# ManuelZ/image-search-engine

Measured on AMD Instinct MI355X. Metric: queries/sec, exact brute-force L2 kNN (recall@10 vs exact CPU), 1Mx512 fp32 index, k=10, higher is better.
Workload: dtype f32; 1 GPU; 1000000x512 fp32 uniform[0,1) index (default_rng 1234), L2, k=10, nq=16 queries per step, index resident in HBM, steps issued round-robin on 16 HIP streams; 400 untimed steps ahead of the warm-up bring the GPU out of its idle power state; n=1000000, d=512, k=10, nq=16

## Files before the change

image-search-engine_amd/_native.py:

```python
from __future__ import annotations

import ctypes
import os

import torch

_HERE = os.path.dirname(os.path.abspath(__file__))
LIB_PATH = os.environ.get("ISE_KNN_LIB") or os.path.join(_HERE, "csrc", "libise_knn.so")

METRIC_INNER_PRODUCT = 0
METRIC_L2 = 1
MAX_K = 2048
PQ_MAX_M = 64
SQ_MAX_D = 2048
SQ_8BIT, SQ_8BIT_UNIFORM = 0, 2
STORE_F32, STORE_BF16 = 0, 1

E_INVALID, E_HIP, E_NOMEM, E_NODEVICE = -1, -2, -3, -4

_f32p = ctypes.POINTER(ctypes.c_float)
_i64p = ctypes.POINTER(ctypes.c_int64)
_u64p = ctypes.POINTER(ctypes.c_uint64)
_vp = ctypes.c_void_p
_i64 = ctypes.c_int64
_int = ctypes.c_int
PROTOTYPES = [
    ("ise_version", _int, []),
    ("ise_last_error", ctypes.c_char_p, []),
    ("ise_device_count", _int, [ctypes.POINTER(_int)]),
    ("ise_device_arch", _int, [_int, ctypes.c_char_p, _int]),
    ("ise_index_create", _int, [ctypes.POINTER(_vp), _int, _int, _int]),
    ("ise_index_create_ex", _int, [ctypes.POINTER(_vp), _int, _int, _int, _int]),
    ("ise_index_destroy", _int, [_vp]),
    ("ise_index_reset", _int, [_vp]),
    ("ise_index_info", _int, [_vp, ctypes.POINTER(_int), ctypes.POINTER(_int), _i64p, ctypes.POINTER(_int)]),
    ("ise_index_set_shift", _int, [_vp, _vp]),
    ("ise_index_get_shift", _int, [_vp, _vp]),
    ("ise_index_stats", _int, [_vp, _u64p]),
    ("ise_index_host_stats", _int, [_vp, _u64p]),
    ("ise_index_reserve_workspaces", _int, [_vp, _i64, _int]),
    ("ise_index_add_host", _int, [_vp, _vp, _i64]),
    ("ise_index_add_device", _int, [_vp, _vp, _i64, _vp]),
    ("ise_index_reconstruct_host", _int, [_vp, _i64, _i64, _vp]),
    ("ise_index_search_host", _int, [_vp, _vp, _i64, _int, _vp, _vp]),
    ("ise_index_search_device", _int, [_vp, _vp, _i64, _int, _vp, _vp, _vp]),
    ("ise_index_search_keys_device", _int, [_vp, _vp, _i64, _int, ctypes.c_uint32, _vp, _vp]),
    ("ise_index_assign_device", _int, [_vp, _vp, _i64, _vp, _vp, _vp]),
    ("ise_merge_keys_device", _int, [_vp, _int, _i64, _int, _int, _vp, _vp, _int, _vp]),
    ("ise_normalize_rows_device", _int, [_vp, _i64, _int, _int, _vp]),
    ("ise_normalize_rows_host", _int, [_vp, _i64, _int, _int]),
    ("ise_bovw_histogram_device", _int, [_vp, _vp, _i64, _int, _vp, _int, _vp]),
    ("ise_index_short_stats", _int, [_vp, _vp]),
    ("ise_index_half_stats", _int, [_vp, _u64p]),
    ("ise_index_shadow_row", _int, [_vp, _i64, _f32p]),
    ("ise_index_byte_stats", _int, [_vp, _u64p]),
    ("ise_index_depth_stats", _int, [_vp, _u64p]),
    ("ise_index_byte_row", _int, [_vp, _i64, _f32p]),
    ("ise_index_stage_query_debug", _int, [_vp, _vp, _int, _vp, _i64, _f32p, ctypes.POINTER(ctypes.c_int32)]),
    ("ise_index_range_search_host", _int, [_vp, _vp, _i64, ctypes.c_float, ctypes.POINTER(_vp)]),
    ("ise_range_result_get", _int, [_vp, _i64p, ctypes.POINTER(_vp), ctypes.POINTER(_vp), ctypes.POINTER(_vp)]),
    ("ise_range_result_destroy", _int, [_vp]),
    ("ise_index_range_stats", _int, [_vp, _u64p]),
    ("ise_index_remove_ids_host", _int, [_vp, _vp, _i64, _i64p]),
    ("ise_index_remove_range", _int, [_vp, _i64, _i64, _i64p]),
    ("ise_index_remove_stats", _int, [_vp, _u64p]),
    ("ise_index_remove_last_timing", _int, [_vp, _f32p, _u64p]),
    ("ise_selector_create_range", _int, [_vp, _i64, _i64, ctypes.POINTER(_vp)]),
    ("ise_selector_create_ids", _int, [_vp, _vp, _i64, _int, ctypes.POINTER(_vp)]),
    ("ise_selector_create_bitmap", _int, [_vp, _vp, _i64, ctypes.POINTER(_vp)]),
    ("ise_selector_info", _int, [_vp, _i64p]),
    ("ise_selector_destroy", _int, [_vp]),
    ("ise_index_search_sel_device", _int, [_vp, _vp, _i64, _int, _vp, _vp, _vp, _vp]),
    ("ise_index_search_sel_host", _int, [_vp, _vp, _i64, _int, _vp, _vp, _vp]),
    ("ise_index_range_search_sel_host", _int, [_vp, _vp, _i64, ctypes.c_float, _vp, ctypes.POINTER(_vp)]),
    ("ise_index_sel_stats", _int, [_vp, _u64p]),
    ("ise_index_search_subset_device", _int, [_vp, _vp, _i64, _int, _vp, _int, _vp, _vp, _vp]),
    ("ise_index_search_subset_host", _int, [_vp, _vp, _i64, _int, _vp, _int, _vp, _vp]),
    ("ise_index_distance_subset_device", _int, [_vp, _vp, _i64, _vp, _int, _vp, _vp]),
    ("ise_index_distance_subset_host", _int, [_vp, _vp, _i64, _vp, _int, _vp]),
    ("ise_index_subset_stats", _int, [_vp, _u64p]),
    ("ise_binary_index_create", _int, [ctypes.POINTER(_vp), _int, _int]),
    ("ise_binary_index_destroy", _int, [_vp]),
    ("ise_binary_index_reset", _int, [_vp]),
    ("ise_binary_index_info", _int, [_vp, ctypes.POINTER(_int), _i64p, ctypes.POINTER(_int)]),
    ("ise_binary_index_add_host", _int, [_vp, _vp, _i64]),
    ("ise_binary_index_add_device", _int, [_vp, _vp, _i64, _vp]),
    ("ise_binary_index_reconstruct_host", _int, [_vp, _i64, _i64, _vp]),
    ("ise_binary_index_search_host", _int, [_vp, _vp, _i64, _int, _vp, _vp]),
    ("ise_binary_index_search_device", _int, [_vp, _vp, _i64, _int, _vp, _vp, _vp]),
    ("ise_binary_index_range_search_host", _int, [_vp, _vp, _i64, ctypes.c_int32, ctypes.POINTER(_vp)]),
    ("ise_binary_range_result_get", _int, [_vp, _i64p, ctypes.POINTER(_vp), ctypes.POINTER(_vp), ctypes.POINTER(_vp)]),
    ("ise_binary_range_result_destroy", _int, [_vp]),
    ("ise_binary_index_stats", _int, [_vp, _u64p]),
    ("ise_binary_index_remove_ids_host", _int, [_vp, _vp, _i64, _i64p]),
    ("ise_binary_index_remove_range", _int, [_vp, _i64, _i64, _i64p]),
    ("ise_binary_index_remove_stats", _int, [_vp, _u64p]),
    ("ise_binary_selector_create_range", _int, [_vp, _i64, _i64, ctypes.POINTER(_vp)]),
    ("ise_binary_selector_create_ids", _int, [_vp, _vp, _i64, _int, ctypes.POINTER(_vp)]),
    ("ise_binary_selector_create_bitmap", _int, [_vp, _vp, _i64, ctypes.POINTER(_vp)]),
    ("ise_binary_selector_info", _int, [_vp, _i64p]),
    ("ise_binary_selector_destroy", _int, [_vp]),
    ("ise_binary_index_search_sel_host", _int, [_vp, _vp, _i64, _int, _vp, _vp, _vp]),
    ("ise_binary_index_search_sel_device", _int, [_vp, _vp, _i64, _int, _vp, _vp, _vp, _vp]),
    ("ise_binary_index_range_search_sel_host", _int, [_vp, _vp, _i64, ctypes.c_int32, _vp, ctypes.POINTER(_vp)]),
    ("ise_binary_index_sel_stats", _int, [_vp, _u64p]),
    ("ise_ivf_create", _int, [ctypes.POINTER(_vp), _int, _int, _int, _int]),
    ("ise_ivf_destroy", _int, [_vp]),
    ("ise_ivf_reset", _int, [_vp]),
    ("ise_ivf_info", _int, [_vp, ctypes.POINTER(_int), ctypes.POINTER(_int), ctypes.POINTER(_int), _i64p, ctypes.POINTER(_int)]),
    ("ise_ivf_add_host", _int, [_vp, _vp, _vp, _i64]),
# ... 82 lines not shown
```

image-search-engine_amd/csrc/ise_knn.hip:

```cpp

#include "ise_host.hpp"
#include "ise_geometry.hpp"
#include "ise_scan_params.hpp"
#include "ise_assign.hpp"
#include "ise_exact.hpp"
#include "ise_merge.hpp"
#include "ise_exact_scan.hpp"
#include "ise_gemm_scan.hpp"
#include "ise_gemm_bf16.hpp"
#include "ise_rows.hpp"
#include "ise_short_scan.hpp"
#include "ise_range.hpp"
#include "ise_sel_scan.hpp"
#include "ise_stage.hpp"
#include "ise_remove.hpp"
#include "ise_remove_plan.hpp"
#include "ise_selector.hpp"
#include "ise_subset.hpp"

static thread_local std::string g_err;
int ise_fail_(int code, const std::string& msg) {
    g_err = msg;
    return code;
}
// ... 280 lines not shown
    }
    h->xb = h->norms = nullptr;
    h->n = h->cap = 0;
}

extern "C" int ise_index_destroy(ise_index_t* h) {
    if (!h) return ISE_OK;
    {
        DeviceGuard gd(h->device);
        (void)hipDeviceSynchronize();
        free_all(h);
        if (h->mu) (void)hipFree(h->mu);
        if (h->stats_dev) (void)hipFree(h->stats_dev);
        if (h->stream) (void)hipStreamDestroy(h->stream);
    }
    delete h;
    return ISE_OK;
}

extern "C" int ise_index_reset(ise_index_t* h) {
    if (!h) return fail(ISE_E_INVALID, "handle is NULL");
    std::lock_guard<std::mutex> lk(h->mu_);
    DeviceGuard gd(h->device);
    HIP_TRY(hipDeviceSynchronize());
    if (h->xb) (void)hipFree(h->xb);
    if (h->norms) (void)hipFree(h->norms);
    free_shadow(h);
    h->shadow_off = false;
    h->byte_off = false;
    if (h->n > 0) h->row_epoch++;
    h->xb = h->norms = nullptr;
    h->n = h->cap = 0;
    h->shift_pinned = false;
    h->mu_rows = h->norms_rows = 0;
    HIP_TRY(hipMemset(h->mu, 0, (size_t)h->dp * sizeof(float)));
    return ISE_OK;
}

extern "C" int ise_index_info(const ise_index_t* h, int* d, int* metric, int64_t* ntotal, int* device) {
    if (!h) return fail(ISE_E_INVALID, "handle is NULL");
    if (d) *d = h->d;
    if (metric) *metric = h->metric;
    if (ntotal) *ntotal = h->n;
    if (device) *device = h->device;
    return ISE_OK;
}

static int reserve_rows(ise_index* h, long long need, hipStream_t st) {
    if (need <= h->cap) return ISE_OK;
    long long cap = h->cap ? h->cap : 0;
    long long want = need;
    if (cap > 0 && want < cap + cap / 2) want = cap + cap / 2;
    want = (want + 15) / 16 * 16;
    const size_t rb = row_bytes(h);
    char* nx = nullptr;
    float* nn = nullptr;
    HIP_TRY(hipMalloc(&nx, (size_t)want * rb));
    hipError_t e = hipMalloc(&nn, (size_t)want * sizeof(float));
    if (e != hipSuccess) {
        (void)hipFree(nx);
        return fail(ISE_E_NOMEM, std::string("hipMalloc(norms): ") + hipGetErrorString(e));
    }
    if (h->n > 0) {
        HIP_TRY(hipMemcpyAsync(nx, h->xb, (size_t)h->n * rb, hipMemcpyDeviceToDevice, st));
        HIP_TRY(hipMemcpyAsync(nn, h->norms, (size_t)h->n * sizeof(float), hipMemcpyDeviceToDevice, st));
    }
    HIP_TRY(hipMemsetAsync(nx + (size_t)h->n * rb, 0, (size_t)(want - h->n) * rb, st));
    HIP_TRY(hipMemsetAsync(nn + h->n, 0, (size_t)(want - h->n) * sizeof(float), st));
    char* nxh = nullptr;
    float* nmeta = nullptr;
    if (h->xh) {
        const size_t hb = shadow_row_bytes(h);
        if (hipMalloc(&nxh, (size_t)want * hb) != hipSuccess || hipMalloc(&nmeta, (size_t)want * 3 * sizeof(float)) != hipSuccess) {
            (void)hipGetLastError();
            if (nxh) (void)hipFree(nxh);
            nxh = nullptr;
        } else {
            HIP_TRY(hipMemcpyAsync(nxh, h->xh, (size_t)h->n * hb, hipMemcpyDeviceToDevice, st));
            HIP_TRY(hipMemsetAsync(nxh + (size_t)h->n * hb, 0, (size_t)(want - h->n) * hb, st));
            HIP_TRY(hipMemsetAsync(nmeta, 0, (size_t)want * 3 * sizeof(float), st));
            for (int i = 0; i < 3; i++)
                HIP_TRY(hipMemcpyAsync(nmeta + (size_t)i * want, h->hmeta + (size_t)i * h->cap, (size_t)h->n * sizeof(float),
                                       hipMemcpyDeviceToDevice, st));
        }
    }
    char* nxq = nullptr;
    uint32_t* nbm = nullptr;
    if (h->xq8 && nxh) {
        const size_t qb = byte_row_bytes(h);
        if (hipMalloc(&nxq, (size_t)want * qb) != hipSuccess || hipMalloc(&nbm, (size_t)want * sizeof(uint32_t)) != hipSuccess) {
            (void)hipGetLastError();
            if (nxq) (void)hipFree(nxq);
            nxq = nullptr;
        } else {
            HIP_TRY(hipMemcpyAsync(nxq, h->xq8, (size_t)h->n * qb, hipMemcpyDeviceToDevice, st));
            HIP_TRY(hipMemsetAsync(nxq + (size_t)h->n * qb, 0, (size_t)(want - h->n) * qb, st));
            HIP_TRY(hipMemsetAsync(nbm, 0, (size_t)want * sizeof(uint32_t), st));
            HIP_TRY(hipMemcpyAsync(nbm, h->bmeta, (size_t)h->n * sizeof(uint32_t), hipMemcpyDeviceToDevice, st));
        }
    }
    HIP_TRY(hipStreamSynchronize(st));
    if (h->xb) HIP_TRY(hipDeviceSynchronize());
    if (h->xb) (void)hipFree(h->xb);
    if (h->norms) (void)hipFree(h->norms);
    if (h->xh) {
        const bool had_byte = h->xq8 != nullptr;
        free_shadow(h);
        h->shadow_off = nxh == nullptr;
        h->byte_off = h->byte_off || (had_byte && nxh && !nxq);
        h->xh = nxh;
        h->hmeta = nmeta;
        h->xq8 = nxq;
        h->bmeta = nbm;
    }
    h->xb = nx;
    h->norms = nn;
    h->cap = want;
    return ISE_OK;
}

static bool rows_copy_verbatim(const ise_index* h) { return h->storage == ISE_STORE_F32 && h->dp == h->d; }

static bool uses_shift(const ise_index* h) { return h->storage == ISE_STORE_F32 && h->metric == ISE_METRIC_L2; }

static int prepare_shift_locked(ise_index* h, hipStream_t st);

static void launch_shadow(ise_index* h, long long row0, long long n, hipStream_t st) {
    const long long nblk = (n + 3) / 4;
    if (nblk > 0)
        hipLaunchKernelGGL(shadow_rows_kernel, dim3((unsigned)nblk), dim3(256), 0, st, (const float*)h->xb, row0, n, h->d,
                           h->dp, (const float*)h->mu, (_Float16*)h->xh, h->dph, h->hmeta, h->hmeta + h->cap,
                           h->hmeta + 2 * h->cap);
    if (nblk > 0 && h->xq8)
        hipLaunchKernelGGL(byte_rows_kernel, dim3((unsigned)nblk), dim3(256), 0, st, (const float*)h->xb, row0, n, h->d,
                           h->dp, (const float*)h->mu, (int8_t*)h->xq8, h->dpb, h->bmeta);
}

static void launch_norms(ise_index* h, long long row0, long long n, hipStream_t st) {
    const long long nblk = (n + 3) / 4;
    if (h->storage == ISE_STORE_BF16)
        hipLaunchKernelGGL(norms_bf16_kernel, dim3((unsigned)nblk), dim3(256), 0, st, (const __bf16*)h->xb, row0, n,
                           h->dp, h->norms);
    else
        hipLaunchKernelGGL(norms_kernel, dim3((unsigned)nblk), dim3(256), 0, st, (const float*)h->xb, row0, n, h->dp,
                           uses_shift(h) ? h->mu : (const float*)nullptr, h->norms);
    if (h->xh) launch_shadow(h, row0, n, st);
}

#define SHADOW_MIN_ROWS 262144
// ... 1961 lines not shown
    hipEvent_t ev0 = nullptr, ev1 = nullptr;
    ~RemoveScratch() {
        for (void* p : {(void*)g, (void*)cend, (void*)src_idx, (void*)bounce})
            if (p) (void)hipFree(p);
        if (ev0) (void)hipEventDestroy(ev0);
        if (ev1) (void)hipEventDestroy(ev1);
    }
};

static void remove_move_rows(const ise_index* h, void* base, size_t stride, long long a, long long m, const RemoveScratch& sc,
                             hipStream_t st) {
    const uint32_t upr = (uint32_t)(stride / 16);
    const uint32_t total = (uint32_t)(m * upr);
    const uint32_t pieces = (total + 64 * REMOVE_UNROLL - 1) / (64 * REMOVE_UNROLL);
    const unsigned grid = std::max(1u, std::min((pieces + 3) / 4, (unsigned)h->num_cu * 4u));
    hipLaunchKernelGGL(remove_rows_kernel<true>, dim3(grid), dim3(256), 0, st, (const u32x4*)base,
                       (const uint32_t*)sc.src_idx, (u32x4*)sc.bounce, total, upr);
    hipLaunchKernelGGL(remove_rows_kernel<false>, dim3(grid), dim3(256), 0, st, (const u32x4*)sc.bounce,
                       (const uint32_t*)nullptr, (u32x4*)(static_cast<char*>(base) + (size_t)a * stride), total, upr);
}

static int remove_runs_locked(ise_index* h, const std::vector<RemoveRun>& runs, long long removed) {
    const long long n_old = h->n, n_new = n_old - removed, first = runs[0].start;
    const long long moved = n_new - first;
    hipStream_t st = h->stream;
    HIP_TRY(hipDeviceSynchronize());
    if (n_new <= SHADOW_MIN_ROWS) free_shadow(h);
    const bool meta = h->norms_rows == n_old;
    const size_t rb = row_bytes(h), hb = shadow_row_bytes(h), qb = byte_row_bytes(h);
    const bool mv_h = meta && h->xh, mv_q = meta && h->xq8;
    RemoveScratch sc;
    if (moved > 0) {
        const long long T = (long long)runs.size();
        std::vector<uint32_t> g, cend;
        remove_plan_tables(runs, &g, &cend);
        const long long slab = remove_plan_slab_rows(ise_remove_slab_rows_(), (long long)rb, (long long)(rb / 16), moved);
        HIP_TRY(hipMalloc(&sc.g, (size_t)T * sizeof(uint32_t)));
        HIP_TRY(hipMalloc(&sc.cend, (size_t)T * sizeof(uint32_t)));
        HIP_TRY(hipMalloc(&sc.src_idx, (size_t)slab * sizeof(uint32_t)));
        HIP_TRY(hipMalloc(&sc.bounce, (size_t)slab * rb));
        HIP_TRY(hipEventCreate(&sc.ev0));
        HIP_TRY(hipEventCreate(&sc.ev1));
        HIP_TRY(hipMemcpyAsync(sc.g, g.data(), (size_t)T * sizeof(uint32_t), hipMemcpyHostToDevice, st));
        HIP_TRY(hipMemcpyAsync(sc.cend, cend.data(), (size_t)T * sizeof(uint32_t), hipMemcpyHostToDevice, st));
        HIP_TRY(hipStreamSynchronize(st));
        HIP_TRY(hipEventRecord(sc.ev0, st));
        for (long long a = first; a < n_new; a += slab) {
            const long long m = std::min(slab, n_new - a);
            const unsigned gw = (unsigned)std::min<long long>((m + 255) / 256, (long long)h->num_cu * 8);
            hipLaunchKernelGGL(remove_src_kernel, dim3(gw), dim3(256), 0, st, (const uint32_t*)sc.g,
                               (const uint32_t*)sc.cend, (int)T, (uint32_t)a, (uint32_t)m, sc.src_idx);
            remove_move_rows(h, h->xb, rb, a, m, sc, st);
            if (mv_h) remove_move_rows(h, h->xh, hb, a, m, sc, st);
            if (mv_q) remove_move_rows(h, h->xq8, qb, a, m, sc, st);
            if (meta) {
                RemovePlanes gp{}, cp{};
                int np = 0;
                auto plane = [&](void* arr) {
                    uint32_t* w = static_cast<uint32_t*>(arr);
                    uint32_t* b = reinterpret_cast<uint32_t*>(sc.bounce) + (size_t)np * m;
                    gp.src[np] = w;
                    gp.dst[np] = b;
                    cp.src[np] = b;
                    cp.dst[np] = w + a;
                    np++;
                };
                plane(h->norms);
                if (mv_h)
                    for (int i = 0; i < 3; i++) plane(h->hmeta + (size_t)i * h->cap);
                if (mv_q) plane(h->bmeta);
                hipLaunchKernelGGL(remove_words_kernel<true>, dim3(gw, np), dim3(256), 0, st, gp,
                                   (const uint32_t*)sc.src_idx, (uint32_t)m);
                hipLaunchKernelGGL(remove_words_kernel<false>, dim3(gw, np), dim3(256), 0, st, cp,
                                   (const uint32_t*)nullptr, (uint32_t)m);
            }
            HIP_TRY(hipGetLastError());
        }
        HIP_TRY(hipEventRecord(sc.ev1, st));
    }
    HIP_TRY(hipMemsetAsync(static_cast<char*>(h->xb) + (size_t)n_new * rb, 0, (size_t)removed * rb, st));
    HIP_TRY(hipMemsetAsync(h->norms + n_new, 0, (size_t)removed * sizeof(float), st));
    if (h->xh) {
        HIP_TRY(hipMemsetAsync(static_cast<char*>(h->xh) + (size_t)n_new * hb, 0, (size_t)removed * hb, st));
        for (int i = 0; i < 3; i++)
            HIP_TRY(hipMemsetAsync(h->hmeta + (size_t)i * h->cap + n_new, 0, (size_t)removed * sizeof(float), st));
    }
    if (h->xq8) {
        HIP_TRY(hipMemsetAsync(static_cast<char*>(h->xq8) + (size_t)n_new * qb, 0, (size_t)removed * qb, st));
        HIP_TRY(hipMemsetAsync(h->bmeta + n_new, 0, (size_t)removed * sizeof(uint32_t), st));
    }
    h->n = n_new;
    h->row_epoch++;
    h->norms_rows = meta ? n_new : 0;
    const long long mu_rows_old = h->mu_rows;
    h->mu_rows = std::min(h->mu_rows, n_new);
    if (uses_shift(h) && !h->shift_pinned && n_new * 4 < mu_rows_old * 3) h->mu_rows = 0;
    HIP_TRY(hipGetLastError());
    HIP_TRY(hipStreamSynchronize(st));
    h->remove_last_ms = 0.f;
    h->remove_last_bytes = 0;
    if (moved > 0) {
        (void)hipEventElapsedTime(&h->remove_last_ms, sc.ev0, sc.ev1);
        const size_t per_row = rb + (mv_h ? hb + 12 : 0) + (mv_q ? qb + 4 : 0) + (meta ? 4 : 0);
        h->remove_last_bytes = (unsigned long long)moved * per_row;
    }
    h->remove_calls++;
    h->remove_rows += (unsigned long long)removed;
    h->remove_moved += (unsigned long long)moved;
    return ISE_OK;
}

extern "C" int ise_index_remove_range(ise_index_t* h, int64_t i0, int64_t i1, int64_t* n_removed) {
    if (!h) return fail(ISE_E_INVALID, "handle is NULL");
    if (n_removed) *n_removed = 0;
    std::lock_guard<std::mutex> lr(h->rg_mu);
    std::lock_guard<std::mutex> lk(h->mu_);
    const long long a = std::max<long long>(i0, 0), b = std::min<long long>(i1, h->n);
    if (a >= b) return ISE_OK;
    DeviceGuard gd(h->device);
    const int rc = remove_runs_locked(h, {RemoveRun{a, b - a}}, b - a);
    if (rc == ISE_OK && n_removed) *n_removed = b - a;
    return rc;
}

extern "C" int ise_index_remove_ids_host(ise_index_t* h, const int64_t* ids, int64_t n_ids, int64_t* n_removed) {
    if (!h) return fail(ISE_E_INVALID, "handle is NULL");
    if (n_removed) *n_removed = 0;
    if (n_ids < 0 || (n_ids > 0 && !ids)) return fail(ISE_E_INVALID, "ids is NULL");
    if (n_ids == 0) return ISE_OK;
    std::vector<long long> v;
    std::vector<RemoveRun> runs;
    try {
        v = remove_plan_ids(ids, n_ids);
    } catch (const std::bad_alloc&) {
        return fail(ISE_E_NOMEM, "remove_ids: host allocation failed");
    }
    std::lock_guard<std::mutex> lr(h->rg_mu);
    std::lock_guard<std::mutex> lk(h->mu_);
    long long removed = 0;
    try {
        removed = remove_plan_runs(v, h->n, &runs);
// ... 29 lines not shown
    std::lock_guard<std::mutex> lk(h->rg_mu);
    out2[0] = h->range_batches;
    out2[1] = h->range_overflows;
    return ISE_OK;
}

extern "C" int ise_index_short_stats(ise_index_t* h, uint64_t* out1) {
    if (!h || !out1) return fail(ISE_E_INVALID, "NULL argument");
    std::lock_guard<std::mutex> lk(h->mu_);
    out1[0] = h->short_batches;
    return ISE_OK;
}

extern "C" int ise_index_depth_stats(ise_index_t* h, uint64_t* out2) {
    if (!h || !out2) return fail(ISE_E_INVALID, "NULL argument");
    std::lock_guard<std::mutex> lk(h->mu_);
    out2[0] = h->byte_batches - h->byte_deep_batches;
    out2[1] = h->byte_deep_batches;
    return ISE_OK;
}

extern "C" int ise_index_half_stats(ise_index_t* h, uint64_t* out1) {
    if (!h || !out1) return fail(ISE_E_INVALID, "NULL argument");
    std::lock_guard<std::mutex> lk(h->mu_);
    out1[0] = h->half_batches;
    return ISE_OK;
}

extern "C" int ise_index_byte_stats(ise_index_t* h, uint64_t* out2) {
    if (!h || !out2) return fail(ISE_E_INVALID, "NULL argument");
    std::lock_guard<std::mutex> lk(h->mu_);
    out2[0] = h->byte_batches;
    out2[1] = (h->xq8 && byte_rel_ok(h)) ? 1 : 0;
    return ISE_OK;
}

extern "C" int ise_index_byte_row(ise_index_t* h, int64_t i, float* out2) {
    if (!h || !out2) return fail(ISE_E_INVALID, "NULL argument");
    std::lock_guard<std::mutex> lk(h->mu_);
    if (i < 0 || i >= h->n) return fail(ISE_E_INVALID, "row out of range");
    DeviceGuard gd(h->device);
    int rc = prepare_shift_locked(h, h->stream);
    if (rc) return rc;
    if (!h->xq8) return fail(ISE_E_INVALID, "this index has no byte shadow rows");
    HIP_TRY(hipDeviceSynchronize());
    uint32_t m = 0;
    HIP_TRY(hipMemcpy(&m, h->bmeta + i, sizeof(uint32_t), hipMemcpyDeviceToHost));
    uint32_t cb = m << 16, eb = m >> 16;
    float cr;
    memcpy(&cr, &cb, sizeof(float));
    const _Float16 eh = __builtin_bit_cast(_Float16, (unsigned short)eb);
    out2[0] = cr;
    out2[1] = cr * (float)eh;
    return ISE_OK;
}

extern "C" int ise_index_shadow_row(ise_index_t* h, int64_t i, float* out3) {
    if (!h || !out3) return fail(ISE_E_INVALID, "NULL argument");
    std::lock_guard<std::mutex> lk(h->mu_);
    if (i < 0 || i >= h->n) return fail(ISE_E_INVALID, "row out of range");
    DeviceGuard gd(h->device);
    int rc = prepare_shift_locked(h, h->stream);
    if (rc) return rc;
    if (!h->xh) return fail(ISE_E_INVALID, "this index has no shadow rows");
    HIP_TRY(hipDeviceSynchronize());
    for (int j = 0; j < 3; j++)
        HIP_TRY(hipMemcpy(out3 + j, h->hmeta + (size_t)j * h->cap + i, sizeof(float), hipMemcpyDeviceToHost));
    return ISE_OK;
}

extern "C" int ise_index_stage_query_debug(ise_index_t* h, const void* q_dev, int route, void* limbs, int64_t limbs_bytes,
                                           float* out2, int32_t* info3) {
    if (!h || !q_dev || !limbs || !out2 || !info3) return fail(ISE_E_INVALID, "NULL argument");
    if (route != 0 && route != 1) return fail(ISE_E_INVALID, "route: 0 = fp16 shadow, 1 = byte shadow");
    std::lock_guard<std::mutex> lk(h->mu_);
    DeviceGuard gd(h->device);
    int rc = prepare_shift_locked(h, h->stream);
    if (rc) return rc;
    if (route == 1 ? !h->xq8 : !h->xh) return fail(ISE_E_INVALID, "this index has no such shadow rows");
    const int P = route == 1 ? h->dpb : h->dph, es = route == 1 ? 1 : 2;
    const size_t need = (size_t)2 * P * es;
    if (P > 1024 || limbs_bytes < (int64_t)need) return fail(ISE_E_INVALID, "limbs: room for hi and lo of the padded row needed");
    unsigned char* dev = nullptr;
    HIP_TRY(hipMalloc(&dev, need + 16));
    float* out_f = reinterpret_cast<float*>(dev + need);
    int* out_i = reinterpret_cast<int*>(dev + need + 8);
    if (route == 1)
        hipLaunchKernelGGL(stage_debug_kernel<true>, dim3(1), dim3(32), 0, h->stream, (const float*)q_dev, h->mu, h->d, P, dev, out_f, out_i);
    else
        hipLaunchKernelGGL(stage_debug_kernel<false>, dim3(1), dim3(32), 0, h->stream, (const float*)q_dev, h->mu, h->d, P, dev, out_f, out_i);
    hipError_t e = hipGetLastError();
    if (e == hipSuccess) e = hipStreamSynchronize(h->stream);
    std::vector<unsigned char> host(need + 16);
    if (e == hipSuccess) e = hipMemcpy(host.data(), dev, need + 16, hipMemcpyDeviceToHost);
    (void)hipFree(dev);
    HIP_TRY(e);
    memcpy(limbs, host.data(), need);
    memcpy(out2, host.data() + need, 8);
    memcpy(info3, host.data() + need + 8, 8);
    info3[2] = P;
    return ISE_OK;
}

extern "C" int ise_index_host_stats(ise_index_t* h, uint64_t* out3) {
    if (!h || !out3) return fail(ISE_E_INVALID, "NULL argument");
    {
// ... 183 lines not shown
```

image-search-engine_amd/csrc/ise_rows.hpp:

```cpp
#pragma once
#include "ise_common.hpp"

__global__ __launch_bounds__(256) void norms_kernel(const float* __restrict__ x, long long row0,
                                                    long long n, int dp, const float* __restrict__ mu,
                                                    float* __restrict__ out) {
    const int lane = threadIdx.x & 63;
    const long long r = row0 + (long long)blockIdx.x * 4 + (threadIdx.x >> 6);
    if (r >= row0 + n) return;
    const float* xr = x + (size_t)r * dp;
    float s = 0.f;
    for (int j = lane * 4; j < dp; j += 256) {
        const f32x4 x = *reinterpret_cast<const f32x4*>(xr + j);
        f32x4 v = x;
        if (mu) v = v - *reinterpret_cast<const f32x4*>(mu + j);
        s = fmaf(v[0], v[0], s);
        s = fmaf(v[1], v[1], s);
        s = fmaf(v[2], v[2], s);
        s = fmaf(v[3], v[3], s);
        if (mu) s += nonfinite_mark(x);
    }
    s = wave_sum_f32(s);
    if (lane == 0) out[r] = s;
}

__global__ __launch_bounds__(256) void shadow_rows_kernel(const float* __restrict__ x, long long row0, long long n,
                                                          int d, int dp, const float* __restrict__ mu,
                                                          _Float16* __restrict__ xh, int dph, float* __restrict__ hn,
                                                          float* __restrict__ he, float* __restrict__ hs) {
    const int lane = threadIdx.x & 63;
    const long long r = row0 + (long long)blockIdx.x * 4 + (threadIdx.x >> 6);
    if (r >= row0 + n) return;
    const float* xr = x + (size_t)r * dp;
    double amax = 0.0;
    float mark = 0.f;
    for (int j = lane; j < d; j += 64) {
        const float v = xr[j];
        mark += v - v;
        amax = fmax(amax, fabs((double)v - (double)mu[j]));
    }
#pragma unroll
    for (int o = 32; o > 0; o >>= 1) {
        amax = fmax(amax, __shfl_xor(amax, o));
        mark += __shfl_xor(mark, o);
    }
    const bool bad = mark != 0.f;
    const int s = (amax > 0.0 && !bad) ? 14 - ilogb(amax) : 0;
    _Float16* hr = xh + (size_t)r * dph;
    double nu = 0.0, e2 = 0.0;
    for (int j = lane; j < dph; j += 64) {
        const double a = (j < d && !bad) ? (double)xr[j] - (double)mu[j] : 0.0;
        const _Float16 u = (_Float16)(float)ldexp(a, s);
        hr[j] = u;
        const double ut = ldexp((double)(float)u, -s);
        nu = fma(ut, ut, nu);
        e2 = fma(a - ut, a - ut, e2);
    }
#pragma unroll
    for (int o = 32; o > 0; o >>= 1) {
        nu += __shfl_xor(nu, o);
        e2 += __shfl_xor(e2, o);
    }
    if (lane == 0) {
        const double e = sqrt(e2) * (1.0 + 0x1p-40) + sqrt(nu) * 0x1p-49;
        float ef = (float)e;
        if ((double)ef < e) ef = nextafterf(ef, INFINITY);
        hn[r] = bad ? __int_as_float(0x7fc00000) : (float)nu;
        he[r] = ef;
        hs[r] = (float)s;
    }
}

__global__ __launch_bounds__(256) void byte_rows_kernel(const float* __restrict__ x, long long row0, long long n,
                                                        int d, int dp, const float* __restrict__ mu,
                                                        int8_t* __restrict__ xq, int dpb, uint32_t* __restrict__ bm) {
    const int lane = threadIdx.x & 63;
    const long long r = row0 + (long long)blockIdx.x * 4 + (threadIdx.x >> 6);
    if (r >= row0 + n) return;
    const float* xr = x + (size_t)r * dp;
    double amax = 0.0;
    float mark = 0.f;
    for (int j = lane; j < d; j += 64) {
        const float v = xr[j];
        mark += v - v;
        amax = fmax(amax, fabs((double)v - (double)mu[j]));
    }
#pragma unroll
    for (int o = 32; o > 0; o >>= 1) {
        amax = fmax(amax, __shfl_xor(amax, o));
        mark += __shfl_xor(mark, o);
    }
    const bool bad = mark != 0.f;
    const double c = bad ? 0.0 : amax / 127.0;
    float cf = (float)c;
    if ((double)cf < c) cf = nextafterf(cf, INFINITY);
    uint32_t cb = __float_as_uint(cf);
    if (cb & 0xFFFFu) cb = (cb + 0x10000u) & 0xFFFF0000u;
    const double cr = (double)__uint_as_float(cb);
    int8_t* qr = xq + (size_t)r * dpb;
    double nu = 0.0, e2 = 0.0;
    for (int j = lane; j < dpb; j += 64) {
        const double a = (j < d && !bad) ? (double)xr[j] - (double)mu[j] : 0.0;
        const double q = cr > 0.0 ? fmin(fmax(rint(a / cr), -127.0), 127.0) : 0.0;
        qr[j] = (int8_t)q;
        const double res = a - cr * q;
        nu = fma(a, a, nu);
        e2 = fma(res, res, e2);
    }
#pragma unroll
    for (int o = 32; o > 0; o >>= 1) {
        nu += __shfl_xor(nu, o);
        e2 += __shfl_xor(e2, o);
    }
    if (lane == 0) {
        const double e = sqrt(e2) * (1.0 + 0x1p-40) + sqrt(nu) * 0x1p-49;
        const double eps = cr > 0.0 ? e / cr * (1.0 + 0x1p-40) : 0.0;
        float ef = (float)eps;
        if ((double)ef < eps) ef = nextafterf(ef, INFINITY);
        unsigned short hb = __builtin_bit_cast(unsigned short, (_Float16)ef);
        if ((float)__builtin_bit_cast(_Float16, hb) < ef) hb++;
        bm[r] = (cb >> 16) | ((uint32_t)hb << 16);
    }
}

__global__ __launch_bounds__(1024) void byte_rel_kernel(const float* __restrict__ norms, const uint32_t* __restrict__ bm,
                                                        long long n, double* __restrict__ out) {
    __shared__ double ss[1024], sc[1024];
    double s = 0.0, cnt = 0.0;
    for (long long i = threadIdx.x; i < n; i += 1024) {
        const float nn = norms[i];
        if (nn > 0.f && nn <= FLT_MAX) {
            const uint32_t m = bm[i];
            const float er = __uint_as_float(m << 16) * (float)__builtin_bit_cast(_Float16, (unsigned short)(m >> 16));
            s += (double)er / sqrt((double)nn);
            cnt += 1.0;
        }
    }
    ss[threadIdx.x] = s;
    sc[threadIdx.x] = cnt;
    __syncthreads();
    for (int o = 512; o > 0; o >>= 1) {
        if ((int)threadIdx.x < o) {
            ss[threadIdx.x] += ss[threadIdx.x + o];
            sc[threadIdx.x] += sc[threadIdx.x + o];
        }
        __syncthreads();
    }
    if (threadIdx.x == 0) out[0] = sc[0] > 0.0 ? ss[0] / sc[0] : 0.0;
}

__global__ __launch_bounds__(256) void sample_dist_kernel(const float* __restrict__ x, int dp, int d, long long stride, int m,
                                                          float* __restrict__ out) {
    const long long t = (long long)blockIdx.x * 256 + threadIdx.x;
    if (t >= (long long)m * m) return;
    const int i = (int)(t / m), j = (int)(t % m);
    const float* a = x + (size_t)i * stride * dp;
    const float* b = x + (size_t)j * stride * dp;
    float s = 0.f;
    for (int c = 0; c < d; c++) s = fmaf(a[c] - b[c], a[c] - b[c], s);
    out[t] = i == j ? INFINITY : s;
}
__global__ __launch_bounds__(1024) void rho_kernel(const float* __restrict__ dist, int m, double* __restrict__ out) {
    __shared__ double sn[1024], sp[1024], cn[1024], cp[1024];
    const int i = threadIdx.x;
    double mn = INFINITY, sum = 0.0, cnt = 0.0;
    if (i < m)
        for (int j = 0; j < m; j++) {
            const float v = dist[(size_t)i * m + j];
            if (v <= FLT_MAX) {
                mn = fmin(mn, (double)v);
                sum += v;
                cnt += 1.0;
            }
        }
    const bool ok = mn <= 1e300;
// ... 198 lines not shown
```

image-search-engine_amd/csrc/ise_scan.hpp:

```cpp
#pragma once
#include "ise_common.hpp"
#include "ise_scan_params.hpp"
#include "ise_select.hpp"
#include "ise_stage.hpp"

#ifndef ISE_FINAL_FILTER
#define ISE_FINAL_FILTER 1
#endif

#ifdef ISE_ABLATE
#define ABL(bit) (p.ablate & (bit))
#define STAMP(i)                                                                                   \
    do {                                                                                           \
        if (p.stamps && lane == 0)                                                                 \
            p.stamps[((size_t)blockIdx.x * W + w) * 16 + (i)] = __builtin_amdgcn_s_memrealtime();  \
    } while (0)
#define CSTAMP(i)                                                                                  \
    do {                                                                                           \
        if (p.stamps && lane == 0)                                                                 \
            p.stamps[((size_t)blockIdx.x * W + w) * 16 + (i)] = __builtin_amdgcn_s_memtime();      \
    } while (0)
#else
#define ABL(bit) 0
#define STAMP(i) do {} while (0)
#define CSTAMP(i) do {} while (0)
#endif

template <int CH, int W, int T, bool BF16, bool SHIFT, int RM = ROWS_OWN>
__global__ __launch_bounds__(W * 64, T == 1 ? W / 2 : (W / 4 > 0 ? W / 4 : 1)) void scan_kernel(const ScanParams p) {
    constexpr bool HALF = RM == ROWS_F16, BYTE = RM == ROWS_I8 || RM == ROWS_I8_ONE, SHADOW = HALF || BYTE;
    static_assert(!(BF16 && SHIFT), "the shift is applied to fp32 rows only");
    static_assert(!SHADOW || SHIFT, "shadow rows belong to float32 L2 indexes");
    constexpr bool F32S = SHIFT && !SHADOW;
    if (p.gate && *p.gate == 0u) return;
    constexpr int BLOCK_THREADS = W * 64;
    constexpr bool XCHG = T >= 3 || (T == 2 && W == 8) || (BYTE && T == 1 && W == 8);
    constexpr bool FFILT = XCHG && ISE_FINAL_FILTER;
    constexpr bool NBOOT = scan_seeded_boot(BYTE, W, T);
    static_assert(!NBOOT || XCHG, "the seeded boot reads the exchange");
    constexpr int NQ = 16 * T;
    constexpr int TPR = W >= 16 ? 32 : BLOCK_THREADS / 16;
    constexpr int KPLB = (W * 16 + 63) / 64;
    constexpr int KPLF = (KB_MAX + W * CAP + 63) / 64;
    static_assert(KB_MAX + CAP <= 64 && MERGE_TRIG + 4 <= CAP, "list sizes");
    extern __shared__ __align__(16) unsigned char smem[];
    const int S = p.qs_stride;
    const int kb = p.kb;
    float* mus = reinterpret_cast<float*>(smem);
    float* qs = mus + S;
    float* xn = qs + NQ * S;
    float* xe = xn + NQ;
    int* xsh = reinterpret_cast<int*>(xe + NQ);
    u64* tauS = reinterpret_cast<u64*>(xn + (SHADOW ? 3 : 1) * NQ);
    int* bwc = reinterpret_cast<int*>(tauS + NQ);
    int* lockS = bwc + NQ;
    int* cntS = lockS + NQ;
    u64* bootw = reinterpret_cast<u64*>(cntS + W * NQ);
    u64* cand = bootw + NQ * kb;
    u64* boot = cand;
    u64* home2 = cand + (size_t)W * NQ * CAP;
    u64* bminS = home2 + (size_t)NQ * W * 16;
    int* arrS = reinterpret_cast<int*>(bminS + NQ);

    const int tid = threadIdx.x, lane = tid & 63, w = __builtin_amdgcn_readfirstlane(tid >> 6);
    const int c = lane & 15, g = lane >> 4;
    const int q0 = blockIdx.y * NQ;
    const int nqt = min(NQ, p.nq - q0);
    const int k = p.k;
    const int nsteps = p.row_slots >> 2;
    const int t0 = blockIdx.x * p.tiles_per_block;
    const int t1 = min(t0 + p.tiles_per_block, p.tiles_total);
    const bool l2 = p.metric == ISE_METRIC_L2;
    STAMP(0);

    auto load_chunk = [&](f32x4(&a)[CH], int tile, int s0) {
        const char* base = static_cast<const char*>(p.xb) +
                           ((((size_t)tile * 16 + c) * p.row_slots + 4 * s0 + g) << 4);
        if (ABL(32)) base = static_cast<const char*>(p.xb) + (((size_t)c * p.row_slots + g) << 4);
        if (ABL(128)) return;
#pragma unroll
        for (int s = 0; s < CH; s++) a[s] = *reinterpret_cast<const f32x4*>(base + 64 * s);
    };
    auto load_norms = [&](int tile) -> f32x4 {
        return *reinterpret_cast<const f32x4*>(p.norms + (size_t)tile * 16 + 4 * g);
    };
    auto load_meta = [&](const void* m, int tile) -> f32x4 {
        if constexpr (!SHADOW) return (f32x4){0.f, 0.f, 0.f, 0.f};
        return *reinterpret_cast<const f32x4*>(static_cast<const float*>(m) + (size_t)tile * 16 + 4 * g);
    };

    constexpr int FPS = BF16 ? 2 : 1;
    constexpr int QV = 8;
    constexpr int QVS = QV / FPS;
    const int S4 = S >> 2;
    const int dslots = BF16 ? (p.d >> 3) : (p.d >> 2);
    const bool vec_q = !SHADOW && (p.d & (BF16 ? 7 : 3)) == 0 && ((reinterpret_cast<uintptr_t>(p.q) & 15) == 0) &&
                       S4 <= TPR * QVS;
    f32x4 qv[T][QV];
    f32x4 muv[F32S ? QVS : 1];
    const bool stager = tid < 16 * TPR;
    if (F32S && vec_q && stager) {
#pragma unroll
        for (int i = 0; i < QVS; i++) {
            const int j4 = tid % TPR + i * TPR;
            muv[i] = (f32x4){0.f, 0.f, 0.f, 0.f};
            if (j4 < dslots) muv[i] = *reinterpret_cast<const f32x4*>(p.mu + 4 * j4);
        }
    }
    if (vec_q && stager) {
#pragma unroll
        for (int tq = 0; tq < T; tq++) {
            const int cc = tq * 16 + tid / TPR, t = tid % TPR;
            const bool rowok = cc < nqt && !ABL(1);
            const float* src = p.q + (size_t)(q0 + (rowok ? cc : 0)) * p.d;
#pragma unroll
            for (int i = 0; i < QVS; i++) {
                const int j4 = t + i * TPR;
#pragma unroll
                for (int f = 0; f < FPS; f++) {
                    qv[tq][i * FPS + f] = (f32x4){0.f, 0.f, 0.f, 0.f};
                    if (rowok && j4 < dslots)
                        qv[tq][i * FPS + f] = *reinterpret_cast<const f32x4*>(src + 4 * (j4 * FPS + f));
                }
            }
        }
    }
    const int PS = p.row_slots * (BYTE ? 16 : 8);
    const bool vec_s = SHADOW && W < 16 && shadow_vec_ok(p.d, PS, p.q, TPR);
    f32x4 sqv[SHADOW ? T : 1][SHADOW_QV], smuv[SHADOW_QV];
    auto shadow_src = [&](int tq) -> const float* {
        const int cc = tq * 16 + tid / TPR;
        return p.q + (size_t)(q0 + ((cc < nqt && !ABL(1)) ? cc : 0)) * p.d;
    };
    if constexpr (SHADOW) {
// ... 684 lines not shown
```

image-search-engine_amd/faiss_compat.py:

```python
from __future__ import annotations

import ctypes
import struct
import threading

import numpy as np

from . import _native as _n

METRIC_INNER_PRODUCT = _n.METRIC_INNER_PRODUCT
METRIC_L2 = _n.METRIC_L2

_FLT_MAX = float(np.finfo(np.float32).max)


def _as_rows(x, d=None) -> np.ndarray:
    x = np.ascontiguousarray(np.asarray(x), dtype=np.float32)
    assert x.ndim == 2, "expected a 2-D array"
    if d is not None:
        assert x.shape[1] == d, f"dimension mismatch: got {x.shape[1]}, index has d={d}"
    return x


def _default_device() -> int:
# ... 271 lines not shown
        finally:
            ds.close()

    def sel_stats(self) -> dict:
        return _counters(self._fn("sel_stats"), self._h, ("sel_batches", "sel_passes", "sel_range_batches"))


class IndexFlat(_RemovableIndex):

    _ABI = "ise_index"
    _FOREIGN_SELECTOR = "a binary index's selector cannot filter a float index"

    def __init__(self, d: int, metric: int = METRIC_L2, device: int | None = None, storage: str = "f32"):
        self.d = int(d)
        self.metric_type = int(metric)
        self.is_trained = True
        self.storage = storage
        self.device = _default_device() if device is None else int(device)
        self._h = ctypes.c_void_p()
        self._lock = threading.Lock()
        store = {"f32": _n.STORE_F32, "bf16": _n.STORE_BF16}[storage]
        _n.check(_n.lib.ise_index_create_ex(ctypes.byref(self._h), self.d, self.metric_type, self.device, store))

    @property
    def ntotal(self) -> int:
        n = ctypes.c_int64(0)
        _n.check(_n.lib.ise_index_info(self._h, None, None, ctypes.byref(n), None))
        return int(n.value)

    def exact_stats(self) -> dict:
        return _counters(_n.lib.ise_index_stats, self._h, ("reranked", "exact_scan", "shift_updates", "gemm_chunks"))

    def host_stats(self) -> dict:
        return _counters(_n.lib.ise_index_host_stats, self._h, ("combined_batches", "combined_calls", "direct_queries"))

    def short_stats(self) -> dict:
        return _counters(_n.lib.ise_index_short_stats, self._h, ("short_batches",))

    def half_stats(self) -> dict:
        return _counters(_n.lib.ise_index_half_stats, self._h, ("half_batches",))

    def byte_stats(self) -> dict:
        c = _counters(_n.lib.ise_index_byte_stats, self._h, ("byte_batches", "byte_route"))
        c["byte_route"] = bool(c["byte_route"])
        return c

    def depth_stats(self) -> dict:
        return _counters(_n.lib.ise_index_depth_stats, self._h, ("isolated_batches", "deep_batches"))

    def byte_row(self, i: int) -> tuple:
        out = (ctypes.c_float * 2)()
        _n.check(_n.lib.ise_index_byte_row(self._h, int(i), out))
        return float(out[0]), float(out[1])

    def shadow_row(self, i: int) -> tuple:
        out = (ctypes.c_float * 3)()
        _n.check(_n.lib.ise_index_shadow_row(self._h, int(i), out))
        return float(out[0]), float(out[1]), int(out[2])

    def stage_query_debug(self, q: "torch.Tensor", route: str) -> dict:
        import torch
        assert q.is_cuda and q.dtype == torch.float32 and q.dim() == 1 and q.is_contiguous() and q.numel() == self.d
        es = {"half": 2, "byte": 1}[route]
        buf = np.zeros(2 * 1024 * es, dtype=np.uint8)
        out, info = (ctypes.c_float * 2)(), (ctypes.c_int32 * 3)()
        torch.cuda.synchronize()
        _n.check(_n.lib.ise_index_stage_query_debug(self._h, q.data_ptr(), es == 1, buf.ctypes.data, buf.nbytes, out, info))
        P = int(info[2])
        limbs = buf[: 2 * P * es].view(np.int8 if es == 1 else np.float16).reshape(2, P)
        return {"hi": limbs[0].copy(), "lo": limbs[1].copy(), "sh": int(info[0]), "vec": bool(info[1]),
                "vn2": float(out[0]), "eq": float(out[1])}

    def range_stats(self) -> dict:
        return _counters(_n.lib.ise_index_range_stats, self._h, ("range_batches", "range_overflow_batches"))

    def reserve(self, nq: int, k: int) -> None:
        _n.check(_n.lib.ise_index_reserve_workspaces(self._h, int(nq), int(k)))

    def get_shift(self) -> np.ndarray:
        mu = np.zeros(self.d, dtype=np.float32)
        _n.check(_n.lib.ise_index_get_shift(self._h, mu.ctypes.data))
        return mu

    def set_shift(self, mu) -> None:
        mu = np.ascontiguousarray(mu, dtype=np.float32)
        assert mu.shape == (self.d,)
        _n.check(_n.lib.ise_index_set_shift(self._h, mu.ctypes.data))

    def add(self, x) -> None:
        x = _as_rows(x, self.d)
        _n.check(_n.lib.ise_index_add_host(self._h, x.ctypes.data, x.shape[0]))

    def add_torch(self, x) -> None:
        import torch

        assert x.is_cuda and x.dtype == torch.float32 and x.dim() == 2 and x.shape[1] == self.d
        x = x.contiguous()
        st = torch.cuda.current_stream(x.device).cuda_stream
        with self._lock:
            _n.check(_n.lib.ise_index_add_device(self._h, x.data_ptr(), x.shape[0], st))
        torch.cuda.current_stream(x.device).synchronize()

    def remove_last_timing(self) -> tuple:
        ms, nb = ctypes.c_float(0), ctypes.c_uint64(0)
        _n.check(_n.lib.ise_index_remove_last_timing(self._h, ctypes.byref(ms), ctypes.byref(nb)))
        return float(ms.value), int(nb.value)
# ... 1532 lines not shown
```

include/ise_knn.h:

```cpp
#ifndef ISE_KNN_H
#define ISE_KNN_H

#include <stdint.h>

#ifdef __cplusplus
extern "C" {
#endif

#define ISE_METRIC_INNER_PRODUCT 0
#define ISE_METRIC_L2 1

#define ISE_STORE_F32 0
#define ISE_STORE_BF16 1

#define ISE_OK 0
#define ISE_E_INVALID -1
#define ISE_E_HIP -2
#define ISE_E_NOMEM -3
#define ISE_E_NODEVICE -4

#define ISE_MAX_K 2048
#define ISE_SQ_MAX_D 2048
#define ISE_PQ_MAX_M 64

typedef struct ise_index ise_index_t;

int ise_version(void);
const char* ise_last_error(void);
int ise_device_count(int* count);
int ise_device_arch(int device, char* buf, int buflen);

int ise_index_create(ise_index_t** out, int d, int metric, int device);
int ise_index_create_ex(ise_index_t** out, int d, int metric, int device, int storage);
int ise_index_destroy(ise_index_t* h);
int ise_index_reset(ise_index_t* h);
int ise_index_info(const ise_index_t* h, int* d, int* metric, int64_t* ntotal, int* device);

int ise_index_add_host(ise_index_t* h, const float* x, int64_t n);
int ise_index_add_device(ise_index_t* h, const float* x_dev, int64_t n, void* stream);

int ise_index_set_shift(ise_index_t* h, const float* mu_host);
int ise_index_get_shift(ise_index_t* h, float* mu_host);

int ise_index_stats(ise_index_t* h, uint64_t* out4);

int ise_index_short_stats(ise_index_t* h, uint64_t* out1);

int ise_index_half_stats(ise_index_t* h, uint64_t* out1);
int ise_index_byte_stats(ise_index_t* h, uint64_t* out2);
int ise_index_depth_stats(ise_index_t* h, uint64_t* out2);
int ise_index_shadow_row(ise_index_t* h, int64_t i, float* out3);
int ise_index_byte_row(ise_index_t* h, int64_t i, float* out2);

int ise_index_stage_query_debug(ise_index_t* h, const void* q_dev, int route, void* limbs, int64_t limbs_bytes,
                                float* out2, int32_t* info3);

int ise_refresh_env_knobs(void);

int ise_index_reserve_workspaces(ise_index_t* h, int64_t nq, int k);

int ise_index_reconstruct_host(ise_index_t* h, int64_t i0, int64_t n, float* out);

int ise_index_search_host(ise_index_t* h, const float* q, int64_t nq, int k,
                          float* D, int64_t* I);
int ise_index_host_stats(ise_index_t* h, uint64_t* out3);

typedef struct ise_range_result ise_range_result_t;
int ise_index_range_search_host(ise_index_t* h, const float* q, int64_t nq, float radius, ise_range_result_t** out);
int ise_range_result_get(const ise_range_result_t* r, int64_t* nq, const int64_t** lims, const float** D,
                         const int64_t** I);
int ise_range_result_destroy(ise_range_result_t* r);
int ise_index_range_stats(ise_index_t* h, uint64_t* out2);

int ise_index_remove_ids_host(ise_index_t* h, const int64_t* ids, int64_t n_ids, int64_t* n_removed);
int ise_index_remove_range(ise_index_t* h, int64_t i0, int64_t i1, int64_t* n_removed);
int ise_index_remove_stats(ise_index_t* h, uint64_t* out3);
int ise_index_remove_last_timing(ise_index_t* h, float* ms, uint64_t* bytes);
int ise_index_search_device(ise_index_t* h, const float* q_dev, int64_t nq, int k,
                            float* D_dev, int64_t* I_dev, void* stream);

typedef struct ise_selector ise_selector_t;
int ise_selector_create_range(ise_index_t* h, int64_t i0, int64_t i1, ise_selector_t** out);
int ise_selector_create_ids(ise_index_t* h, const int64_t* ids_host, int64_t n_ids, int invert, ise_selector_t** out);
int ise_selector_create_bitmap(ise_index_t* h, const uint32_t* words_host, int64_t n_words, ise_selector_t** out);
int ise_selector_info(const ise_selector_t* sel, int64_t* out5);
int ise_selector_destroy(ise_selector_t* sel);
int ise_index_search_sel_device(ise_index_t* h, const float* q_dev, int64_t nq, int k, const ise_selector_t* sel,
                                float* D_dev, int64_t* I_dev, void* stream);
int ise_index_search_sel_host(ise_index_t* h, const float* q, int64_t nq, int k, const ise_selector_t* sel, float* D,
                              int64_t* I);
int ise_index_range_search_sel_host(ise_index_t* h, const float* q, int64_t nq, float radius, const ise_selector_t* sel,
                                    ise_range_result_t** out);
int ise_index_sel_stats(ise_index_t* h, uint64_t* out3);

int ise_index_search_subset_device(ise_index_t* h, const float* q_dev, int64_t nq, int k, const int64_t* cand_dev, int kc,
                                   float* D_dev, int64_t* I_dev, void* stream);
int ise_index_search_subset_host(ise_index_t* h, const float* q, int64_t nq, int k, const int64_t* cand, int kc, float* D,
                                 int64_t* I);
int ise_index_distance_subset_device(ise_index_t* h, const float* q_dev, int64_t nq, const int64_t* cand_dev, int kc,
                                     float* dist_dev, void* stream);
int ise_index_distance_subset_host(ise_index_t* h, const float* q, int64_t nq, const int64_t* cand, int kc, float* dist);
int ise_index_subset_stats(ise_index_t* h, uint64_t* out3);

#define ISE_BINARY_MAX_BITS 8192
typedef struct ise_binary_index ise_binary_index_t;
// ... 124 lines not shown
```

Baseline: 177,100 queries/s.

## Store int8 byte-shadow rows in 16-row tiled layout for coalesced scan loads

Changes the int8 shadow copy of the index from row-major to a 16-row tiled layout in which each 16-byte unit of 16 consecutive rows is contiguous. The scan kernel's chunk loads become fully contiguous per wavefront (stride 1024 per step) and use nontemporal loads for the int8 route. The encode, remove, zero and grow paths are updated to the tiled layout, and a debug accessor for a row's codes is added. The aim is better memory coalescing for the bandwidth-bound byte pre-filter scan. In exchange, row moves during removal now re-encode rows from the fp32 data instead of copying them.

```diff
diff --git a/image-search-engine_amd/_native.py b/image-search-engine_amd/_native.py
--- a/image-search-engine_amd/_native.py
+++ b/image-search-engine_amd/_native.py
@@ -56,6 +56,7 @@
     ("ise_index_byte_stats", _int, [_vp, _u64p]),
     ("ise_index_depth_stats", _int, [_vp, _u64p]),
     ("ise_index_byte_row", _int, [_vp, _i64, _f32p]),
+    ("ise_index_byte_row_codes", _int, [_vp, _i64, _vp]),
     ("ise_index_stage_query_debug", _int, [_vp, _vp, _int, _vp, _i64, _f32p, ctypes.POINTER(ctypes.c_int32)]),
     ("ise_index_range_search_host", _int, [_vp, _vp, _i64, ctypes.c_float, ctypes.POINTER(_vp)]),
     ("ise_range_result_get", _int, [_vp, _i64p, ctypes.POINTER(_vp), ctypes.POINTER(_vp), ctypes.POINTER(_vp)]),
diff --git a/image-search-engine_amd/csrc/ise_byte_layout.hpp b/image-search-engine_amd/csrc/ise_byte_layout.hpp
--- /dev/null
+++ b/image-search-engine_amd/csrc/ise_byte_layout.hpp
@@ -0,0 +1,16 @@
+#pragma once
+#include <cstddef>
+
+#if defined(__HIPCC__) || defined(__CUDACC__)
+#define ISE_BYTE_HD __host__ __device__
+#else
+#define ISE_BYTE_HD
+#endif
+
+constexpr int BYTE_TILE_ROWS = 16;
+
+ISE_BYTE_HD inline size_t byte_unit_index(long long row, int u, int upr) {
+    const size_t tile = (size_t)(row >> 4);
+    const int r = (int)(row & 15);
+    return tile * 16 * (size_t)upr + (size_t)(u >> 2) * 64 + (size_t)(u & 3) * 16 + (size_t)r;
+}
diff --git a/image-search-engine_amd/csrc/ise_knn.hip b/image-search-engine_amd/csrc/ise_knn.hip
--- a/image-search-engine_amd/csrc/ise_knn.hip
+++ b/image-search-engine_amd/csrc/ise_knn.hip
@@ -356,6 +356,7 @@
     long long want = need;
     if (cap > 0 && want < cap + cap / 2) want = cap + cap / 2;
     want = (want + 15) / 16 * 16;
+    static_assert(BYTE_TILE_ROWS == 16, "capacities are whole row tiles: the byte rows are stored and copied by the tile");
     const size_t rb = row_bytes(h);
     char* nx = nullptr;
     float* nn = nullptr;
@@ -397,8 +398,9 @@
             if (nxq) (void)hipFree(nxq);
             nxq = nullptr;
         } else {
-            HIP_TRY(hipMemcpyAsync(nxq, h->xq8, (size_t)h->n * qb, hipMemcpyDeviceToDevice, st));
-            HIP_TRY(hipMemsetAsync(nxq + (size_t)h->n * qb, 0, (size_t)(want - h->n) * qb, st));
+            const long long nt = (h->n + BYTE_TILE_ROWS - 1) / BYTE_TILE_ROWS * BYTE_TILE_ROWS;
+            HIP_TRY(hipMemcpyAsync(nxq, h->xq8, (size_t)nt * qb, hipMemcpyDeviceToDevice, st));
+            HIP_TRY(hipMemsetAsync(nxq + (size_t)nt * qb, 0, (size_t)(want - nt) * qb, st));
             HIP_TRY(hipMemsetAsync(nbm, 0, (size_t)want * sizeof(uint32_t), st));
             HIP_TRY(hipMemcpyAsync(nbm, h->bmeta, (size_t)h->n * sizeof(uint32_t), hipMemcpyDeviceToDevice, st));
         }
@@ -2466,7 +2468,6 @@
                                (const uint32_t*)sc.cend, (int)T, (uint32_t)a, (uint32_t)m, sc.src_idx);
             remove_move_rows(h, h->xb, rb, a, m, sc, st);
             if (mv_h) remove_move_rows(h, h->xh, hb, a, m, sc, st);
-            if (mv_q) remove_move_rows(h, h->xq8, qb, a, m, sc, st);
             if (meta) {
                 RemovePlanes gp{}, cp{};
                 int np = 0;
@@ -2482,7 +2483,6 @@
                 plane(h->norms);
                 if (mv_h)
                     for (int i = 0; i < 3; i++) plane(h->hmeta + (size_t)i * h->cap);
-                if (mv_q) plane(h->bmeta);
                 hipLaunchKernelGGL(remove_words_kernel<true>, dim3(gw, np), dim3(256), 0, st, gp,
                                    (const uint32_t*)sc.src_idx, (uint32_t)m);
                 hipLaunchKernelGGL(remove_words_kernel<false>, dim3(gw, np), dim3(256), 0, st, cp,
@@ -2490,6 +2490,9 @@
             }
             HIP_TRY(hipGetLastError());
         }
+        if (mv_q)
+            hipLaunchKernelGGL(byte_rows_kernel, dim3((unsigned)((moved + 3) / 4)), dim3(256), 0, st, (const float*)h->xb,
+                               first, moved, h->d, h->dp, (const float*)h->mu, (int8_t*)h->xq8, h->dpb, h->bmeta);
         HIP_TRY(hipEventRecord(sc.ev1, st));
     }
     HIP_TRY(hipMemsetAsync(static_cast<char*>(h->xb) + (size_t)n_new * rb, 0, (size_t)removed * rb, st));
@@ -2500,7 +2503,15 @@
             HIP_TRY(hipMemsetAsync(h->hmeta + (size_t)i * h->cap + n_new, 0, (size_t)removed * sizeof(float), st));
     }
     if (h->xq8) {
-        HIP_TRY(hipMemsetAsync(static_cast<char*>(h->xq8) + (size_t)n_new * qb, 0, (size_t)removed * qb, st));
+        const long long upr = (long long)(qb / 16);
+        const long long t_new = (n_new + BYTE_TILE_ROWS - 1) / BYTE_TILE_ROWS * BYTE_TILE_ROWS;
+        const long long t_old = (n_old + BYTE_TILE_ROWS - 1) / BYTE_TILE_ROWS * BYTE_TILE_ROWS;
+        const long long z1 = std::min(t_new, n_old);
+        if (z1 > n_new)
+            hipLaunchKernelGGL(byte_rows_zero_kernel, dim3((unsigned)(((z1 - n_new) * upr + 255) / 256)), dim3(256), 0, st,
+                               (int8_t*)h->xq8, n_new, z1, (int)upr);
+        if (t_old > t_new)
+            HIP_TRY(hipMemsetAsync(static_cast<char*>(h->xq8) + (size_t)t_new * qb, 0, (size_t)(t_old - t_new) * qb, st));
         HIP_TRY(hipMemsetAsync(h->bmeta + n_new, 0, (size_t)removed * sizeof(uint32_t), st));
     }
     h->n = n_new;
@@ -2636,6 +2647,26 @@
     const _Float16 eh = __builtin_bit_cast(_Float16, (unsigned short)eb);
     out2[0] = cr;
     out2[1] = cr * (float)eh;
+    return ISE_OK;
+}
+
+extern "C" int ise_index_byte_row_codes(ise_index_t* h, int64_t i, int8_t* out_dpb) {
+    if (!h || !out_dpb) return fail(ISE_E_INVALID, "NULL argument");
+    std::lock_guard<std::mutex> lk(h->mu_);
+    DeviceGuard gd(h->device);
+    int rc = prepare_shift_locked(h, h->stream);
+    if (rc) return rc;
+    if (!h->xq8) return fail(ISE_E_INVALID, "this index has no byte shadow rows");
+    if (i < 0 || i >= h->cap) return fail(ISE_E_INVALID, "row out of range");
+    HIP_TRY(hipDeviceSynchronize());
+    u32x4* tmp = nullptr;
+    HIP_TRY(hipMalloc(&tmp, (size_t)h->dpb));
+    hipLaunchKernelGGL(byte_row_read_kernel, dim3(1), dim3(64), 0, h->stream, (const int8_t*)h->xq8, (long long)i,
+                       (int)(h->dpb / 16), tmp);
+    hipError_t e = hipMemcpyAsync(out_dpb, tmp, (size_t)h->dpb, hipMemcpyDeviceToHost, h->stream);
+    if (e == hipSuccess) e = hipStreamSynchronize(h->stream);
+    (void)hipFree(tmp);
+    HIP_TRY(e);
     return ISE_OK;
 }
 
diff --git a/image-search-engine_amd/csrc/ise_rows.hpp b/image-search-engine_amd/csrc/ise_rows.hpp
--- a/image-search-engine_amd/csrc/ise_rows.hpp
+++ b/image-search-engine_amd/csrc/ise_rows.hpp
@@ -1,5 +1,6 @@
 #pragma once
 #include "ise_common.hpp"
+#include "ise_byte_layout.hpp"
 
 __global__ __launch_bounds__(256) void norms_kernel(const float* __restrict__ x, long long row0,
                                                     long long n, int dp, const float* __restrict__ mu,
@@ -96,12 +97,20 @@
     uint32_t cb = __float_as_uint(cf);
     if (cb & 0xFFFFu) cb = (cb + 0x10000u) & 0xFFFF0000u;
     const double cr = (double)__uint_as_float(cb);
-    int8_t* qr = xq + (size_t)r * dpb;
+    const int upr = dpb >> 4;
     double nu = 0.0, e2 = 0.0;
     for (int j = lane; j < dpb; j += 64) {
         const double a = (j < d && !bad) ? (double)xr[j] - (double)mu[j] : 0.0;
         const double q = cr > 0.0 ? fmin(fmax(rint(a / cr), -127.0), 127.0) : 0.0;
-        qr[j] = (int8_t)q;
+        const uint32_t b = (uint32_t)(uint8_t)(int8_t)q;
+        const uint32_t w4 = b | (__shfl_down(b, 1) << 8) | (__shfl_down(b, 2) << 16) | (__shfl_down(b, 3) << 24);
+        u32x4 unit;
+        unit[0] = w4;
+        unit[1] = __shfl_down(w4, 4);
+        unit[2] = __shfl_down(w4, 8);
+        unit[3] = __shfl_down(w4, 12);
+        if ((lane & 15) == 0)
+            *reinterpret_cast<u32x4*>(xq + (byte_unit_index(r, j >> 4, upr) << 4)) = unit;
         const double res = a - cr * q;
         nu = fma(a, a, nu);
         e2 = fma(res, res, e2);
@@ -120,6 +129,21 @@
         if ((float)__builtin_bit_cast(_Float16, hb) < ef) hb++;
         bm[r] = (cb >> 16) | ((uint32_t)hb << 16);
     }
+}
+
+__global__ __launch_bounds__(256) void byte_rows_zero_kernel(int8_t* __restrict__ xq, long long row0, long long row1,
+                                                             int upr) {
+    const long long i = (long long)blockIdx.x * 256 + threadIdx.x;
+    const long long row = row0 + i / upr;
+    if (row >= row1) return;
+    const u32x4 z = {0u, 0u, 0u, 0u};
+    *reinterpret_cast<u32x4*>(xq + (byte_unit_index(row, (int)(i % upr), upr) << 4)) = z;
+}
+
+__global__ __launch_bounds__(64) void byte_row_read_kernel(const int8_t* __restrict__ xq, long long row, int upr,
+                                                           u32x4* __restrict__ out) {
+    for (int u = threadIdx.x; u < upr; u += 64)
+        out[u] = *reinterpret_cast<const u32x4*>(xq + (byte_unit_index(row, u, upr) << 4));
 }
 
 __global__ __launch_bounds__(1024) void byte_rel_kernel(const float* __restrict__ norms, const uint32_t* __restrict__ bm,
diff --git a/image-search-engine_amd/csrc/ise_scan.hpp b/image-search-engine_amd/csrc/ise_scan.hpp
--- a/image-search-engine_amd/csrc/ise_scan.hpp
+++ b/image-search-engine_amd/csrc/ise_scan.hpp
@@ -1,6 +1,7 @@
 #pragma once
 #include "ise_common.hpp"
 #include "ise_scan_params.hpp"
+#include "ise_byte_layout.hpp"
 #include "ise_select.hpp"
 #include "ise_stage.hpp"
 
@@ -74,12 +75,19 @@
     STAMP(0);
 
     auto load_chunk = [&](f32x4(&a)[CH], int tile, int s0) {
+        constexpr bool BLOCKED = BYTE;
+        constexpr bool NT = RM == ROWS_I8;
+        constexpr int STEP = BLOCKED ? 1024 : 64;
         const char* base = static_cast<const char*>(p.xb) +
-                           ((((size_t)tile * 16 + c) * p.row_slots + 4 * s0 + g) << 4);
+                           (BLOCKED ? (((size_t)tile * 16 * p.row_slots + (size_t)s0 * 64 + lane) << 4)
+                                    : ((((size_t)tile * 16 + c) * p.row_slots + 4 * s0 + g) << 4));
         if (ABL(32)) base = static_cast<const char*>(p.xb) + (((size_t)c * p.row_slots + g) << 4);
         if (ABL(128)) return;
 #pragma unroll
-        for (int s = 0; s < CH; s++) a[s] = *reinterpret_cast<const f32x4*>(base + 64 * s);
+        for (int s = 0; s < CH; s++) {
+            const f32x4* src = reinterpret_cast<const f32x4*>(base + STEP * s);
+            a[s] = NT ? __builtin_nontemporal_load(src) : *src;
+        }
     };
     auto load_norms = [&](int tile) -> f32x4 {
         return *reinterpret_cast<const f32x4*>(p.norms + (size_t)tile * 16 + 4 * g);
diff --git a/image-search-engine_amd/faiss_compat.py b/image-search-engine_amd/faiss_compat.py
--- a/image-search-engine_amd/faiss_compat.py
+++ b/image-search-engine_amd/faiss_compat.py
@@ -347,6 +347,12 @@
         out = (ctypes.c_float * 2)()
         _n.check(_n.lib.ise_index_byte_row(self._h, int(i), out))
         return float(out[0]), float(out[1])
+
+    def byte_row_codes(self, i: int):
+        steps = (self.d + 63) // 64
+        out = np.zeros((steps if steps <= 4 else (steps + 3) // 4 * 4) * 64, dtype=np.int8)
+        _n.check(_n.lib.ise_index_byte_row_codes(self._h, int(i), out.ctypes.data_as(ctypes.c_void_p)))
+        return out
 
     def shadow_row(self, i: int) -> tuple:
         out = (ctypes.c_float * 3)()
diff --git a/include/ise_knn.h b/include/ise_knn.h
--- a/include/ise_knn.h
+++ b/include/ise_knn.h
@@ -51,6 +51,7 @@
 int ise_index_depth_stats(ise_index_t* h, uint64_t* out2);
 int ise_index_shadow_row(ise_index_t* h, int64_t i, float* out3);
 int ise_index_byte_row(ise_index_t* h, int64_t i, float* out2);
+int ise_index_byte_row_codes(ise_index_t* h, int64_t i, int8_t* out_dpb);
 
 int ise_index_stage_query_debug(ise_index_t* h, const void* q_dev, int route, void* limbs, int64_t limbs_bytes,
                                 float* out2, int32_t* info3);
```

After: 181,100 queries/s (median of 6 runs). 1.02x the previous value.
